# hongsukchoi/Pose2Mesh_RELEASE

Measured on NVIDIA H100. Metric: SMPL meshes/sec, higher is better.
Workload: dtype f32 (wgmma fp16x3 split, fp32 accumulate)

## Files before the change

### pose2mesh_release_b200/csrc/cheb_umma.cu

```cuda
#include <cuda.h>
#include <cuda_fp16.h>
#include <cuda_runtime.h>

#include <algorithm>
#include <cstdlib>
#include <cstring>
#include <vector>

#include "p2m_internal.h"

namespace p2m {

namespace {

constexpr int TILE_M = 128;
constexpr int FC = 32;
constexpr int A_BLOCK_BYTES = TILE_M * 128;
constexpr float W_SCALE = 64.f;
constexpr float W_INV_SCALE = 1.f / 64.f;

struct TileHeader {
  int n_rows;
  int h1;
  int nnz;
  int off_halo;
  int off_rp;
  int off_ent;
  int off_ord2;
  int bytes;
  int pad[8];
};
static_assert(sizeof(TileHeader) == 64, "header size");

inline int up16(int x) { return (x + 15) & ~15; }

constexpr int STG_ROW_BYTES = 544;

__device__ __forceinline__ uint32_t smem_u32(const void* p) { return (uint32_t)__cvta_generic_to_shared(p); }

__device__ __forceinline__ void mbar_init(uint32_t bar, uint32_t count) {
  asm volatile("mbarrier.init.shared::cta.b64 [%0], %1;" ::"r"(bar), "r"(count));
}
__device__ __forceinline__ void mbar_arrive(uint32_t bar) {
  asm volatile("mbarrier.arrive.shared::cta.b64 _, [%0];" ::"r"(bar) : "memory");
}
__device__ __forceinline__ void mbar_arrive_expect_tx(uint32_t bar, uint32_t bytes) {
  asm volatile("mbarrier.arrive.expect_tx.shared::cta.b64 _, [%0], %1;" ::"r"(bar), "r"(bytes) : "memory");
}
__device__ __forceinline__ bool mbar_try_wait(uint32_t bar, uint32_t parity) {
  uint32_t ok;
  asm volatile(
      "{\n\t.reg .pred p;\n\t"
      "mbarrier.try_wait.parity.shared::cta.b64 p, [%1], %2, %3;\n\t"
      "selp.u32 %0, 1, 0, p;\n\t}"
      : "=r"(ok)
      : "r"(bar), "r"(parity), "r"(20000u)
      : "memory");
  return ok != 0;
}
__device__ __forceinline__ unsigned long long global_ns() {
  unsigned long long t;
  asm volatile("mov.u64 %0, %globaltimer;" : "=l"(t));
  return t;
}
constexpr unsigned long long MBAR_TIMEOUT_NS = 2000000000ull;
__device__ __noinline__ void mbar_timeout(volatile int* abort_flag, int* status, int code) {
  *abort_flag = 1;
  *reinterpret_cast<volatile int*>(status) = code;
  __threadfence_system();
}
__device__ __forceinline__ void mbar_wait(uint32_t bar, uint32_t parity, volatile int* abort_flag, int* status,
                                          int code) {
  if (mbar_try_wait(bar, parity)) return;
  unsigned long long t0 = 0;
  for (unsigned spin = 0;; ++spin) {
#pragma unroll 1
    for (int it = 0; it < 64; ++it) {
      if (mbar_try_wait(bar, parity)) return;
    }
    if (*abort_flag) return;
    if ((spin & 63u) == 63u) {
      const unsigned long long t = global_ns();
      if (t0 == 0) t0 = t;
      else if (t - t0 > MBAR_TIMEOUT_NS) break;
    }
  }
  mbar_timeout(abort_flag, status, code);
}
template <unsigned SLEEP_NS = 200>
__device__ __forceinline__ void mbar_wait_relaxed(uint32_t bar, uint32_t parity, volatile int* abort_flag, int* status,
                                                  int code) {
  if (mbar_try_wait(bar, parity)) return;
  unsigned long long t0 = 0;
  for (unsigned spin = 0;; ++spin) {
#pragma unroll 1
    for (int it = 0; it < 16; ++it) {
      if (mbar_try_wait(bar, parity)) return;
      __nanosleep(SLEEP_NS);
    }
    if (*abort_flag) return;
    if ((spin & 255u) == 255u) {
      const unsigned long long t = global_ns();
      if (t0 == 0) t0 = t;
      else if (t - t0 > MBAR_TIMEOUT_NS) break;
    }
  }
  mbar_timeout(abort_flag, status, code);
}
__device__ __forceinline__ void fence_barrier_init() { asm volatile("fence.mbarrier_init.release.cluster;" ::: "memory"); }
// ... 141 lines not shown
__device__ __forceinline__ void split4(const float4& v, uint2& hi, uint2& lo) {
  __half2 h0 = __floats2half2_rn(v.x, v.y), h1 = __floats2half2_rn(v.z, v.w);
  float2 f0 = __half22float2(h0), f1 = __half22float2(h1);
  __half2 l0 = __floats2half2_rn(v.x - f0.x, v.y - f0.y), l1 = __floats2half2_rn(v.z - f1.x, v.w - f1.y);
  hi.x = *reinterpret_cast<uint32_t*>(&h0);
  hi.y = *reinterpret_cast<uint32_t*>(&h1);
  lo.x = *reinterpret_cast<uint32_t*>(&l0);
  lo.y = *reinterpret_cast<uint32_t*>(&l1);
}

struct KParams {
  const float* x;
  int in_unpool;
  int V, P, fin;
  int n_tiles;
  const unsigned char* meta;
  const int* meta_bytes;
  int meta_stride, max_h1;
  const unsigned char* wpack;
  const float* zero_row;
  EpiDev ep;
  int res_identity;
  const float* t1;
  const float* a_scale;
  long long ldy;
  int y_col0;
  float* y;
  int* status;
  long long* trace;
  int own_table;
  const float* head_wt;
  float* head_z;
  const unsigned char* apack;
  long long wslice_bytes;
  long long wblock_stride;
  int tma;
  CUtensorMap tm_x, tm_t1;
};

#ifdef P2M_UMMA_TRACE
__device__ __forceinline__ void trace_ev(const KParams& p, int role, int& n, int ev) {
  if (p.trace != nullptr && blockIdx.x == 0 && blockIdx.y == 0 && n < 512) {
    p.trace[role * 512 + n] = ((long long)ev << 48) | (clock64() & 0xFFFFFFFFFFFFll);
    ++n;
  }
}
#else
__device__ __forceinline__ void trace_ev(const KParams&, int, int&, int) {}
#endif

constexpr int W_PROD = 16;
constexpr int W_XLOAD = 16, N_XLOAD = 2, W_BLOAD = 18, W_EPI0 = 20;
constexpr int NUM_THREADS2 = 24 * 32;
constexpr int REGS_LAUNCH = 80, REGS_UTIL = 40, REGS_EPI = 120;
static_assert(128 * (REGS_EPI - REGS_LAUNCH) <= 128 * (REGS_LAUNCH - REGS_UTIL), "register pool balance");
static_assert(W_XLOAD % 4 == 0 && W_EPI0 % 4 == 0 && W_EPI0 - W_XLOAD == 4, "setmaxnreg works on aligned warpgroups");

template <int N>
__host__ __device__ constexpr int tile_rows() { return N == 128 ? 64 : TILE_M; }
template <int N, int NS, int XS, int MODE>
__global__ void __launch_bounds__(NUM_THREADS2, 1) k_cheb_conv_umma(const __grid_constant__ KParams p) {
  static_assert(N == 64 || N == 128, "one warpgroup holds the CTA's 128 x 64 or 64 x 128 accumulator in registers");
  constexpr int TM = tile_rows<N>();
  constexpr int RPT = TM / 64;
  constexpr int H = TM / 64;
  constexpr int ER = 16 * H;
  constexpr bool KT1 = (MODE == 1);
  constexpr bool plain = !KT1;
  constexpr bool XDIRECT = KT1 && NS >= 3;
  constexpr int A_BYTES = TM * 128;
  constexpr int B_BLOCK_BYTES = N * 128;
  constexpr int SLOT_BYTES = A_BYTES + B_BLOCK_BYTES;

  extern __shared__ __align__(1024) unsigned char smem_raw[];
  unsigned char* ring = smem_raw;
  float* Xs = reinterpret_cast<float*>(ring + NS * SLOT_BYTES);
  const size_t xs_stage_floats = (XDIRECT && TM == 64) ? 0 : (size_t)TM * FC;
  float* T1s = Xs + XS * xs_stage_floats;
  const size_t t1_stage_floats = (size_t)p.max_h1 * FC;
  unsigned char* meta_s =
      reinterpret_cast<unsigned char*>(T1s + (plain ? 0 : XS) * t1_stage_floats);
  uint64_t* bars = reinterpret_cast<uint64_t*>(meta_s + 2 * (size_t)p.meta_stride);
  uint64_t* b_ab_full = bars;
  uint64_t* b_ab_empty = b_ab_full + NS;
  uint64_t* b_x_full = b_ab_empty + NS;
  uint64_t* b_x_empty = b_x_full + XS;
  uint64_t* b_m_full = b_x_empty + XS;
  uint64_t* b_m_empty = b_m_full + 2;
  uint32_t* flags = reinterpret_cast<uint32_t*>(b_m_empty + 2);
  volatile int* abort_flag = reinterpret_cast<volatile int*>(flags + 1);
  float* ep_mul = reinterpret_cast<float*>(flags + 4);
  float* ep_add = ep_mul + N;
  constexpr int EC = 32;
  constexpr int STG_WARP_BYTES = N == 128 ? 16 * STG_ROW_BYTES : 32 * EC * 4;
  unsigned char* epi_stage =
      reinterpret_cast<unsigned char*>((reinterpret_cast<uintptr_t>(ep_add + N) + 127) & ~(uintptr_t)127);
  int* own_s = reinterpret_cast<int*>(epi_stage + 4 * STG_WARP_BYTES);
  float* head_w_s = reinterpret_cast<float*>(own_s + 4 * 32);
  uint64_t* b_res = reinterpret_cast<uint64_t*>(head_w_s);

  const int tid = threadIdx.x;
  const int warp = tid >> 5;
  const int lane = tid & 31;
  const int n_chunk = p.fin / FC;
  const int n_use = 3 * n_chunk;

  if (tid == 0) {
    for (int s = 0; s < NS; ++s) {
      mbar_init(smem_u32(b_ab_full + s), p.apack != nullptr ? 1 : W_PROD + 1);
      mbar_init(smem_u32(b_ab_empty + s), 4);
    }
    for (int s = 0; s < XS; ++s) {
      mbar_init(smem_u32(b_x_full + s), N_XLOAD * 32 + 1);
      mbar_init(smem_u32(b_x_empty + s), 1);
    }
    for (int s = 0; s < 2; ++s) {
      mbar_init(smem_u32(b_m_full + s), 1);
      mbar_init(smem_u32(b_m_empty + s), 1);
    }
    if (N == 128)
      for (int w = 0; w < 4; ++w) mbar_init(smem_u32(b_res + w), 1);
    *abort_flag = (smem_u32(ring) & 1023u) ? 1 : 0;
    if (*abort_flag) mbar_timeout(abort_flag, p.status, 100);
    fence_barrier_init();
  }
  const float a_scale = p.a_scale ? *p.a_scale : 1.f;
  const int ecol0 = (int)blockIdx.y * N;
  for (int n = threadIdx.x; n < N; n += NUM_THREADS2) {
    const float sc = (p.ep.scale ? p.ep.scale[ecol0 + n] : 1.f) / a_scale;
    const float sh = p.ep.scale ? p.ep.shift[ecol0 + n] : 0.f;
    const float bi = p.ep.bias ? p.ep.bias[ecol0 + n] : 0.f;
    ep_mul[n] = W_INV_SCALE * sc;
    ep_add[n] = fmaf(bi, p.ep.scale ? p.ep.scale[ecol0 + n] : 1.f, sh);
  }
  if (N == 64 && p.head_z != nullptr)
    for (int i = threadIdx.x; i < 64 * 12; i += NUM_THREADS2) head_w_s[i] = p.head_wt[i];
  __syncthreads();

  if (warp >= W_XLOAD && warp < W_EPI0) {
  asm volatile("setmaxnreg.dec.sync.aligned.u32 %0;" ::"n"(REGS_UTIL));
  if (warp >= W_XLOAD && warp < W_XLOAD + N_XLOAD) {
    if (p.apack == nullptr) {
      const int lt = tid - W_XLOAD * 32;
      const int lq = lt & 7, lrg = lt >> 3;
      const int my_tiles = (p.n_tiles - (int)blockIdx.x + (int)gridDim.x - 1) / (int)gridDim.x;
      if (lt == 32 && p.tma) {
        if (!XDIRECT) asm volatile("prefetch.tensormap [%0];" ::"l"(reinterpret_cast<uint64_t>(&p.tm_x)) : "memory");
        if (KT1) asm volatile("prefetch.tensormap [%0];" ::"l"(reinterpret_cast<uint64_t>(&p.tm_t1)) : "memory");
      }
      auto fetch_meta = [&](int itf) {
        const int pat = (blockIdx.x + itf * gridDim.x) % p.P;
        const int m = itf & 1;
        mbar_wait_relaxed(smem_u32(b_m_empty + m), ((itf >> 1) & 1) ^ 1, abort_flag, p.status, 1);
        const int mbytes = p.meta_bytes[pat];
        mbar_arrive_expect_tx(smem_u32(b_m_full + m), mbytes);
        bulk_g2s(smem_u32(meta_s + (size_t)m * p.meta_stride), p.meta + (size_t)pat * p.meta_stride, mbytes,
                 smem_u32(b_m_full + m));
      };
      if (lt == 0 && my_tiles > 0) fetch_meta(0);
      const uint32_t fin_bytes = (uint32_t)p.fin * 4u;
      const int sh = p.in_unpool ? 1 : 0;
      int g2 = 0;
      int ltn = 0;
      for (int it2 = 0; it2 < my_tiles; ++it2) {
        const int tile2 = blockIdx.x + it2 * gridDim.x;
        const long long mesh_row0 = (long long)(tile2 / p.P) * p.V;
        const int m2 = it2 & 1;
        mbar_wait_relaxed(smem_u32(b_m_full + m2), (it2 >> 1) & 1, abort_flag, p.status, 8);
        const unsigned char* mb2 = meta_s + (size_t)m2 * p.meta_stride;
        const TileHeader* hdr2 = reinterpret_cast<const TileHeader*>(mb2);
        const int* halo = reinterpret_cast<const int*>(mb2 + hdr2->off_halo);
        const int h1 = hdr2->h1;
        for (int c2 = 0; c2 < n_chunk; ++c2, ++g2) {
          const int xs2 = g2 % XS;
          mbar_wait_relaxed(smem_u32(b_x_empty + xs2), ((g2 / XS) & 1) ^ 1, abort_flag, p.status, 11);
          if (lt == 0) trace_ev(p, 4, ltn, 1);
          const uint32_t xbar = smem_u32(b_x_full + xs2);
          auto stage_rows = [&](uint32_t dbase, const char* sbase, int first, int n_rows, int shift) {
            for (int i0 = first + lrg; i0 < n_rows; i0 += 32) {
              int v[4];
#pragma unroll
              for (int u = 0; u < 4; ++u) v[u] = (i0 + 8 * u < n_rows) ? halo[i0 + 8 * u] : -2;
#pragma unroll
              for (int u = 0; u < 4; ++u) {
                if (v[u] != -2) {
                  const uint32_t srow = (uint32_t)max(v[u], 0) >> shift;
                  cp_async16_zfill(dbase + (i0 + 8 * u) * 128, sbase + (uint64_t)srow * (uint64_t)fin_bytes,
                                   v[u] >= 0 ? 16u : 0u);
                }
              }
            }
          };
          const char* t1_mesh =
              reinterpret_cast<const char*>(KT1 ? p.t1 + mesh_row0 * p.fin + c2 * FC + lq * 4 : nullptr);
          const char* x_mesh = reinterpret_cast<const char*>(p.x + (mesh_row0 >> sh) * p.fin + c2 * FC + lq * 4);
          const uint32_t t1_dst = smem_u32(T1s + xs2 * t1_stage_floats) + lq * 16;
          const uint32_t x_dst = smem_u32(Xs + xs2 * xs_stage_floats) + lq * 16;
          if (p.tma) {
            if (lt == 32) {
              const int own0 = tile2 * TM;
              mbar_arrive_expect_tx(xbar, (XDIRECT ? 0 : (p.in_unpool ? TM / 2 : TM) * 128) + (KT1 ? TM * 128 : 0));
              if (!XDIRECT)
                tma_load_2d(smem_u32(Xs + xs2 * xs_stage_floats), &p.tm_x, c2 * FC, p.in_unpool ? own0 >> 1 : own0, xbar);
              if (KT1) tma_load_2d(smem_u32(T1s + xs2 * t1_stage_floats), &p.tm_t1, c2 * FC, own0, xbar);
            }
            if (KT1) stage_rows(t1_dst, t1_mesh, TM, h1, 0);
          } else {
            if (KT1) stage_rows(t1_dst, t1_mesh, 0, h1, 0);
            if (!XDIRECT) stage_rows(x_dst, x_mesh, 0, TM, sh);
            if (lt == 32) mbar_arrive(xbar);
          }
          cp_async_arrive_noinc(xbar);
          if (lt == 0) trace_ev(p, 4, ltn, 2);
          if (lt == 0 && c2 == (n_chunk > 1 ? 1 : 0) && it2 + 1 < my_tiles) fetch_meta(it2 + 1);
        }
      }
    }
  } else if (warp == W_BLOAD) {
    if (lane == 0) {
      uint32_t ucnt = 0;
      int tn = 0;
      const int uses = plain ? n_chunk : n_use;
      for (int tile = blockIdx.x; tile < p.n_tiles; tile += gridDim.x) {
        for (int u = 0; u < uses; ++u, ++ucnt) {
          const int s = ucnt % NS;
          const uint32_t par = (ucnt / NS) & 1;
          mbar_wait_relaxed(smem_u32(b_ab_empty + s), par ^ 1, abort_flag, p.status, 4);
          trace_ev(p, 1, tn, 10 + u);
          const unsigned char* wsl = p.wpack + (size_t)blockIdx.y * (size_t)p.wslice_bytes;
          if (p.apack != nullptr) {
            mbar_arrive_expect_tx(smem_u32(b_ab_full + s), B_BLOCK_BYTES + A_BYTES);
            bulk_g2s(smem_u32(ring + s * SLOT_BYTES), p.apack + ((size_t)tile * uses + u) * A_BYTES, A_BYTES,
                     smem_u32(b_ab_full + s));
          } else {
            mbar_arrive_expect_tx(smem_u32(b_ab_full + s), B_BLOCK_BYTES);
          }
          bulk_g2s(smem_u32(ring + s * SLOT_BYTES + A_BYTES), wsl + (size_t)u * (size_t)p.wblock_stride, B_BLOCK_BYTES,
                   smem_u32(b_ab_full + s));
        }
      }
    }
  }
  } else if (warp >= W_EPI0) {
    asm volatile("setmaxnreg.inc.sync.aligned.u32 %0;" ::"n"(REGS_EPI));
    const int wq = warp - W_EPI0;
    constexpr int CPR = EC / 4;
    constexpr int RPI = 32 / CPR;
    const uint32_t stg = smem_u32(epi_stage) + (uint32_t)wq * STG_WARP_BYTES;
    const int prow = lane / CPR, pc = lane % CPR;
    constexpr int NP = ER / RPI;
    int colk[2];
#pragma unroll
    for (int k = 0; k < 2; ++k) colk[k] = (int)(((uint32_t)pc ^ (uint32_t)((k * RPI + prow) & 7)) << 2);
    const int trow = (lane >> 4) * 64 + wq * 16 + (lane & 15);
    const int uses = plain ? n_chunk : n_use;
    uint32_t ucnt = 0;
    int it = 0;
    int etn = 0;
    for (int tile = blockIdx.x; tile < p.n_tiles; tile += gridDim.x, ++it) {
      const int b = tile / p.P, pat = tile - b * p.P;
      const long long mesh0 = (long long)b * p.V;
      int* own_w = own_s + wq * 32;
      {
        int v;
        if (lane >= ER) {
          v = -1;
        } else if (p.own_table) {
          v = __ldg(reinterpret_cast<const int*>(p.meta + (size_t)pat * p.meta_stride + 64) + trow);
        } else {
          v = pat * TM + trow;
          if (v >= p.V) v = -1;
        }
        __syncwarp();
        own_w[lane] = v;
        __syncwarp();
      }
      int own_v[NP];
#pragma unroll
      for (int i = 0; i < NP; ++i) own_v[i] = own_w[i * RPI + prow];
      if (N == 128) {
        if (lane < ER) bulk_wait_read0();
        __syncwarp();
        if (p.ep.res != nullptr && p.res_identity) {
          const uint32_t rbar = smem_u32(b_res + wq);
          const int n_valid = __popc(__ballot_sync(0xFFFFFFFFu, lane < ER && own_w[lane] >= 0));
          if (lane == 0) mbar_arrive_expect_tx(rbar, (uint32_t)n_valid * (N * 4));
          __syncwarp();
          if (lane < ER && own_w[lane] >= 0) {
            const long long r = mesh0 + own_w[lane];
            bulk_g2s(stg + lane * STG_ROW_BYTES, p.ep.res + (p.ep.res_unpool ? (r >> 1) : r) * p.ep.res_F + ecol0, N * 4,
                     rbar);
          }
        }
      }
      if (p.ep.res != nullptr && (N == 64 || !p.res_identity)) {
        const int lpr = ((p.apack != nullptr ? N : p.ep.res_F) * 4 + 127) >> 7;
        for (int j = lane; j < ER * lpr; j += 32) {
          const int rr = j / lpr, ln = j - rr * lpr;
          const int vtx = own_w[rr];
          if (vtx >= 0) {
            const long long r = mesh0 + vtx;
            prefetch_l2(p.ep.res + (p.ep.res_unpool ? (r >> 1) : r) * p.ep.res_F + (p.apack != nullptr ? ecol0 : 0) + ln * 32);
          }
        }
      }
      float acc[2][32];
#pragma unroll
      for (int h = 0; h < 2; ++h)
#pragma unroll
        for (int j = 0; j < 32; ++j) acc[h][j] = 0.f;
      if (wq == 0 && lane == 0) trace_ev(p, 3, etn, 1);
      for (int u = 0; u < uses; ++u, ++ucnt) {
        const uint32_t s = ucnt % NS;
        if (wq == 0 && lane == 0) trace_ev(p, 3, etn, 4);
        mbar_wait(smem_u32(b_ab_full + s), (ucnt / NS) & 1, abort_flag, p.status, 6);
        if (wq == 0 && lane == 0) trace_ev(p, 3, etn, 5);
        const uint32_t a0 = smem_u32(ring + s * SLOT_BYTES);
        wg_fence();
#pragma unroll
        for (int h = 0; h < 2; ++h) {
          const uint64_t da = make_desc_sw128(a0 + (TM == 128 ? (uint32_t)h * (64 * 128) : 0u));
          const uint64_t db = make_desc_sw128(a0 + A_BYTES + (TM == 64 ? (uint32_t)h * (64 * 128) : 0u));
          wgmma_m64n64<0, 0>(acc[h], da + 0, db + 0);
          wgmma_m64n64<0, 0>(acc[h], da + 2, db + 2);
          wgmma_m64n64<0, 0>(acc[h], da + 4, db + 0);
          wgmma_m64n64<0, 0>(acc[h], da + 6, db + 2);
          wgmma_m64n64<0, 0>(acc[h], da + 0, db + 4);
          wgmma_m64n64<0, 0>(acc[h], da + 2, db + 6);
        }
        wg_commit();
        wg_wait0();
        __syncwarp();
        if (lane == 0) mbar_arrive(smem_u32(b_ab_empty + s));
      }
      if (wq == 0 && lane == 0) trace_ev(p, 3, etn, 2);
      auto stage_slab = [&](int cb) {
#pragma unroll
        for (int h = 0; h < H; ++h)
#pragma unroll
          for (int jj = 0; jj < 4; ++jj)
#pragma unroll
            for (int r = 0; r < 2; ++r) {
              const int lr = 16 * h + (lane >> 2) + 8 * r;
              const int cc = 8 * jj + 2 * (lane & 3);
              const int j = 4 * (cb / 8 + jj) + 2 * r;
              sts_f2(stg + lr * (EC * 4) + ((((uint32_t)(cc >> 2)) ^ (uint32_t)(lr & 7)) << 4) + (cc & 3) * 4,
                     acc[h][j], acc[h][j + 1]);
            }
        __syncwarp();
      };
      if (N == 64 && p.head_z != nullptr) {
        float z[12];
#pragma unroll
        for (int j = 0; j < 12; ++j) z[j] = 0.f;
#pragma unroll
        for (int cb = 0; cb < N; cb += 32) {
          stage_slab(cb);
#pragma unroll
          for (int c = 0; c < 8; ++c) {
            const float4 a = lds_f4(stg + lane * (EC * 4) + (((uint32_t)c ^ (uint32_t)(lane & 7)) << 4));
            const float av[4] = {a.x, a.y, a.z, a.w};
#pragma unroll
            for (int e = 0; e < 4; ++e) {
              const int n = cb + 4 * c + e;
              float t = fmaf(av[e], ep_mul[n], ep_add[n]);
              if (p.ep.relu) t = fmaxf(t, 0.f);
              const float4 w0 = *reinterpret_cast<const float4*>(head_w_s + n * 12);
              const float4 w1 = *reinterpret_cast<const float4*>(head_w_s + n * 12 + 4);
              const float4 w2 = *reinterpret_cast<const float4*>(head_w_s + n * 12 + 8);
              z[0] = fmaf(t, w0.x, z[0]); z[1] = fmaf(t, w0.y, z[1]); z[2] = fmaf(t, w0.z, z[2]); z[3] = fmaf(t, w0.w, z[3]);
              z[4] = fmaf(t, w1.x, z[4]); z[5] = fmaf(t, w1.y, z[5]); z[6] = fmaf(t, w1.z, z[6]); z[7] = fmaf(t, w1.w, z[7]);
              z[8] = fmaf(t, w2.x, z[8]); z[9] = fmaf(t, w2.y, z[9]); z[10] = fmaf(t, w2.z, z[10]); z[11] = fmaf(t, w2.w, z[11]);
            }
          }
          __syncwarp();
        }
        if (own_w[lane] >= 0) {
          float4* zr = reinterpret_cast<float4*>(p.head_z + (mesh0 + own_w[lane]) * 12);
          zr[0] = make_float4(z[0], z[1], z[2], z[3]);
          zr[1] = make_float4(z[4], z[5], z[6], z[7]);
          zr[2] = make_float4(z[8], z[9], z[10], z[11]);
        }
      } else if (N == 128) {
        const bool res_id = p.ep.res != nullptr && p.res_identity;
        if (res_id) mbar_wait(smem_u32(b_res + wq), (uint32_t)it & 1u, abort_flag, p.status, 12);
        if (wq == 0 && lane == 0) trace_ev(p, 3, etn, 21);
#pragma unroll
        for (int h = 0; h < 2; ++h)
#pragma unroll
          for (int jg = 0; jg < 8; ++jg) {
            const int n = 64 * h + 8 * jg + 2 * (lane & 3);
            const float2 mu = *reinterpret_cast<const float2*>(ep_mul + n);
            const float2 ad = *reinterpret_cast<const float2*>(ep_add + n);
#pragma unroll
            for (int r = 0; r < 2; ++r) {
              const int j = 4 * jg + 2 * r;
              const uint32_t a = stg + ((lane >> 2) + 8 * r) * STG_ROW_BYTES + n * 4;
              float o0 = fmaf(acc[h][j], mu.x, ad.x), o1 = fmaf(acc[h][j + 1], mu.y, ad.y);
              if (p.ep.relu) {
                o0 = fmaxf(o0, 0.f);
                o1 = fmaxf(o1, 0.f);
              }
              if (res_id) {
                const float2 rv = lds_f2(a);
                o0 += rv.x;
                o1 += rv.y;
              }
              sts_f2(a, o0, o1);
            }
          }
        if (p.ep.res != nullptr && !p.res_identity) {
          __syncwarp();
          const int gn = ecol0 + 4 * lane;
          for (int rr = 0; rr < ER; ++rr) {
            const int vtx = own_w[rr];
            if (vtx >= 0) {
              const long long r = mesh0 + vtx;
              const float* res_row = p.ep.res + (p.ep.res_unpool ? (r >> 1) : r) * p.ep.res_F;
              const uint32_t a = stg + rr * STG_ROW_BYTES + lane * 16;
              const float4 v = lds_f4(a);
              float o[4] = {v.x, v.y, v.z, v.w};
#pragma unroll
              for (int e = 0; e < 4; ++e) {
                const float l = __ldg(p.ep.lam + gn + e);
                o[e] += (1.f - l) * __ldg(res_row + __ldg(p.ep.i0 + gn + e)) + l * __ldg(res_row + __ldg(p.ep.i1 + gn + e));
              }
              sts_f4(a, make_float4(o[0], o[1], o[2], o[3]));
            }
          }
        }
        if (wq == 0 && lane == 0) trace_ev(p, 3, etn, 22);
        fence_async_proxy();
        __syncwarp();
        if (lane < ER) {
          if (own_w[lane] >= 0)
            bulk_s2g(p.y + (mesh0 + own_w[lane]) * p.ldy + p.y_col0 + ecol0, stg + lane * STG_ROW_BYTES, N * 4);
          bulk_commit();
        }
        if (wq == 0 && lane == 0) trace_ev(p, 3, etn, 23);
      } else {
#pragma unroll
        for (int cb = 0; cb < N; cb += 32) {
          stage_slab(cb);
          float4 mu_k[2], ad_k[2];
#pragma unroll
          for (int k = 0; k < 2; ++k) {
            mu_k[k] = *reinterpret_cast<const float4*>(ep_mul + cb + colk[k]);
            ad_k[k] = *reinterpret_cast<const float4*>(ep_add + cb + colk[k]);
          }
#pragma unroll
          for (int i = 0; i < NP; ++i) {
            const int rr = i * RPI + prow;
            const int n = cb + colk[i & 1];
            const int gn = ecol0 + n;
            const float4 a = lds_f4(stg + rr * (EC * 4) + (pc << 4));
            const int vtx = own_v[i];
            if (vtx >= 0) {
              const float4 mu = mu_k[i & 1], ad = ad_k[i & 1];
              float o[4] = {fmaf(a.x, mu.x, ad.x), fmaf(a.y, mu.y, ad.y), fmaf(a.z, mu.z, ad.z), fmaf(a.w, mu.w, ad.w)};
              if (p.ep.relu) {
#pragma unroll
                for (int e = 0; e < 4; ++e) o[e] = fmaxf(o[e], 0.f);
              }
              const long long r = mesh0 + vtx;
              if (p.ep.res != nullptr) {
                const float* res_row = p.ep.res + (p.ep.res_unpool ? (r >> 1) : r) * p.ep.res_F;
                if (p.res_identity) {
                  const float4 rv = __ldg(reinterpret_cast<const float4*>(res_row + gn));
                  o[0] += rv.x; o[1] += rv.y; o[2] += rv.z; o[3] += rv.w;
                } else {
#pragma unroll
                  for (int e = 0; e < 4; ++e) {
                    const float l = __ldg(p.ep.lam + gn + e);
                    o[e] += (1.f - l) * __ldg(res_row + __ldg(p.ep.i0 + gn + e)) + l * __ldg(res_row + __ldg(p.ep.i1 + gn + e));
                  }
                }
              }
              *reinterpret_cast<float4*>(p.y + r * p.ldy + p.y_col0 + gn) = make_float4(o[0], o[1], o[2], o[3]);
            }
          }
          __syncwarp();
        }
      }
    }
    if (N == 128 && lane < ER) bulk_wait0();
  } else {
    if (p.apack == nullptr) {
    const int q = tid & 7;
    const int rg = tid >> 3;
    const uint32_t t1s_a = smem_u32(T1s);
    const uint32_t ring_a = smem_u32(ring);
    const int my_tiles = (p.n_tiles - (int)blockIdx.x + (int)gridDim.x - 1) / (int)gridDim.x;
    const int n_stage = my_tiles * n_chunk;

    uint32_t row[RPT], re[RPT], ent_a = 0;
    int ptn = 0;
    uint32_t slot = 0, spar = 0;
    uint32_t so_f[RPT], so_s[RPT];
#pragma unroll
    for (int ps = 0; ps < RPT; ++ps) row[ps] = re[ps] = so_f[ps] = so_s[ps] = 0;
    const bool odd = (rg & 1) != 0;
    auto next_slot = [&]() {
      if (++slot == (uint32_t)NS) {
        slot = 0;
        spar ^= 1u;
      }
    };

    const int xsh = (p.tma && p.in_unpool) ? 1 : 0;
    const float* xp[RPT];
#pragma unroll
    for (int ps = 0; ps < RPT; ++ps) xp[ps] = nullptr;
    int it = 0, c = -1;
    for (int g = 0; g < n_stage; ++g) {
      if (++c == n_chunk) {
        c = 0;
        ++it;
      }
      const int m = it & 1;
      const int xs = g % XS;
      float4 xd[RPT];
#pragma unroll
      for (int ps = 0; ps < RPT; ++ps) {
        xd[ps] = make_float4(0.f, 0.f, 0.f, 0.f);
        if (XDIRECT && c != 0 && xp[ps]) xd[ps] = __ldg(reinterpret_cast<const float4*>(xp[ps] + c * FC));
      }
      if (tid == 0) trace_ev(p, 0, ptn, 1);
      mbar_wait(smem_u32(b_x_full + xs), (g / XS) & 1, abort_flag, p.status, 9);
      if (tid == 0) trace_ev(p, 0, ptn, 2);

      if (c == 0) {
        mbar_wait(smem_u32(b_m_full + m), (it >> 1) & 1, abort_flag, p.status, 8);
        const unsigned char* mb = meta_s + (size_t)m * p.meta_stride;
        const TileHeader* hdr = reinterpret_cast<const TileHeader*>(mb);
        const uint32_t mb_a = smem_u32(mb);
        const uint32_t rp_a = mb_a + hdr->off_rp, ord2_a = mb_a + hdr->off_ord2;
        ent_a = mb_a + hdr->off_ent;
#pragma unroll
        for (int ps = 0; ps < RPT; ++ps) {
// ... 67 lines not shown
      };
      float4 x[RPT], t1v[RPT], t2[RPT];
      if (NS < 3) {
#pragma unroll
        for (int ps = 0; ps < RPT; ++ps) x[ps] = lds_f4(xs_q + (row[ps] >> xsh) * 128);
        emit(x);
#pragma unroll
        for (int ps = 0; ps < RPT; ++ps) t1v[ps] = lds_f4(t1s_q + row[ps] * 128);
        emit(t1v);
#pragma unroll
        for (int ps = 0; ps < RPT; ++ps) t2[ps] = gather_row4(ent_a, re[ps] & 0xFFFFu, re[ps] >> 16, t1s_q);
        if (tid == 0) trace_ev(p, 0, ptn, 6);
#pragma unroll
        for (int ps = 0; ps < RPT; ++ps) t2[ps] = cheb_t2(t2[ps], x[ps]);
        emit(t2);
      } else {
#pragma unroll
        for (int ps = 0; ps < RPT; ++ps) t2[ps] = gather_row4(ent_a, re[ps] & 0xFFFFu, re[ps] >> 16, t1s_q);
#pragma unroll
        for (int ps = 0; ps < RPT; ++ps) x[ps] = XDIRECT ? xd[ps] : lds_f4(xs_q + (row[ps] >> xsh) * 128);
#pragma unroll
        for (int ps = 0; ps < RPT; ++ps) t1v[ps] = lds_f4(t1s_q + row[ps] * 128);
        if (tid == 0) trace_ev(p, 0, ptn, 6);
        {
          uint32_t s2 = slot + 2, p2 = spar;
          if (s2 >= (uint32_t)NS) {
            s2 -= (uint32_t)NS;
            p2 ^= 1u;
          }
          mbar_wait(smem_u32(b_ab_empty + s2), p2 ^ 1u, abort_flag, p.status, 10);
        }
        emit(x);
        emit(t1v);
#pragma unroll
        for (int ps = 0; ps < RPT; ++ps) t2[ps] = cheb_t2(t2[ps], x[ps]);
        emit(t2);
      }
      if (NS >= 3) {
        fence_async_proxy();
        __syncwarp();
        if ((tid & 31) == 0) {
#pragma unroll
          for (int k = 0; k < 3; ++k) mbar_arrive(smem_u32(b_ab_full + (slot0 + k) % NS));
        }
      }
      if (tid == 0) trace_ev(p, 0, ptn, 7);
      producer_barrier();
      if (tid == 0) trace_ev(p, 0, ptn, 8);
      if (tid == 0) mbar_arrive(smem_u32(b_x_empty + xs));
      if (tid == 0 && c == n_chunk - 1) mbar_arrive(smem_u32(b_m_empty + m));
    }
    }
  }
}

struct DwParams {
  const float* x;
  int in_unpool;
  int V, P, fin;
  int n_tiles;
  const unsigned char* meta;
  const int* meta_bytes;
  int meta_stride, max_h1;
  const float* g;
  int fout_total, m_off, m_cols;
  int chunk0;
  const float* a_scale;
  float* dw;
  int* status;
  const float* t1;
  int g_unpool;
  int swap;
  int tma;
  CUtensorMap tm_x, tm_t1;
};

__device__ __forceinline__ uint64_t make_desc_sw128_mn(uint32_t saddr, uint32_t lbo_bytes) {
  uint64_t d = 0;
  d |= (uint64_t)((saddr & 0x3FFFF) >> 4);
  d |= (uint64_t)((lbo_bytes >> 4) & 0x3FFF) << 16;
  d |= (uint64_t)(1024 >> 4) << 32;
  d |= (uint64_t)1 << 62;
  return d;
}

constexpr int DW_NS = 3;
constexpr int DW_G_BYTES = 4 * A_BLOCK_BYTES;

template <int XS>
__global__ void __launch_bounds__(NUM_THREADS2, 1) k_cheb_dw_umma(const __grid_constant__ DwParams p) {
  extern __shared__ __align__(1024) unsigned char smem_raw[];
  unsigned char* ring = smem_raw;
  unsigned char* gblk = ring + DW_NS * A_BLOCK_BYTES;
  float* Xs = reinterpret_cast<float*>(gblk + DW_G_BYTES);
  constexpr size_t xs_stage_floats = (size_t)TILE_M * FC;
  float* T1s = Xs + XS * xs_stage_floats;
  const size_t t1_stage_floats = (size_t)p.max_h1 * FC;
  unsigned char* meta_s = reinterpret_cast<unsigned char*>(T1s + XS * t1_stage_floats);
  uint64_t* bars = reinterpret_cast<uint64_t*>(meta_s + 2 * (size_t)p.meta_stride);
  uint64_t* b_t_full = bars;
  uint64_t* b_t_empty = b_t_full + DW_NS;
  uint64_t* b_x_full = b_t_empty + DW_NS;
  uint64_t* b_x_empty = b_x_full + XS;
  uint64_t* b_m_full = b_x_empty + XS;
  uint64_t* b_m_empty = b_m_full + 2;
  uint64_t* b_g_full = b_m_empty + 2;
// ... 386 lines not shown
}
size_t smem_bytes_for(int N, int NS, int XS, const TileBlobs& t, bool t1_given) {
  return smem_bytes_dims(N, NS, XS, t.max_h1, t.stride, t1_given);
}
constexpr size_t SMEM_LIMIT = 227 * 1024;
constexpr int CONV_N = 64;
constexpr int WIDE_N = 128;
inline int conv_n(int fout) { return fout % WIDE_N == 0 ? WIDE_N : CONV_N; }
const TileBlobs& conv_tiles(int N, const DevLevel& g, const TileSet* tiles) {
  if (tiles != nullptr) return N == WIDE_N ? tiles->m64 : *tiles;
  return N == WIDE_N ? g.meta64 : g.meta128;
}
struct ConvCfg {
  int ns, xs;
};
ConvCfg conv_cfg(int N, const TileBlobs& t, bool t1_given) {
  for (int ns = N == WIDE_N ? 6 : 3; ns >= 3; ns -= 3)
    for (int xs = 2; xs >= 1; --xs)
      if (smem_bytes_for(N, ns, xs, t, t1_given) <= SMEM_LIMIT) return {ns, xs};
  return {0, 0};
}

typedef CUresult (*TmapEncodeFn)(CUtensorMap*, CUtensorMapDataType, cuuint32_t, void*, const cuuint64_t*, const cuuint64_t*,
                                 const cuuint32_t*, const cuuint32_t*, CUtensorMapInterleave, CUtensorMapSwizzle,
                                 CUtensorMapL2promotion, CUtensorMapFloatOOBfill);
TmapEncodeFn tmap_encoder() {
  static TmapEncodeFn fn = [] {
    void* f = nullptr;
    cudaDriverEntryPointQueryResult q;
    if (cudaGetDriverEntryPoint("cuTensorMapEncodeTiled", &f, cudaEnableDefault, &q) != cudaSuccess ||
        q != cudaDriverEntryPointSuccess)
      f = nullptr;
    return reinterpret_cast<TmapEncodeFn>(f);
  }();
  return fn;
}
bool make_row_tmap(CUtensorMap* tm, const float* base, long long rows, int fin, int box_rows) {
  TmapEncodeFn enc = tmap_encoder();
  if (enc == nullptr || (reinterpret_cast<uintptr_t>(base) & 15u) != 0) return false;
  const cuuint64_t dims[2] = {(cuuint64_t)fin, (cuuint64_t)rows};
  const cuuint64_t strides[1] = {(cuuint64_t)fin * 4};
  const cuuint32_t box[2] = {(cuuint32_t)FC, (cuuint32_t)box_rows};
  const cuuint32_t estr[2] = {1, 1};
  return enc(tm, CU_TENSOR_MAP_DATA_TYPE_FLOAT32, 2, const_cast<float*>(base), dims, strides, box, estr,
             CU_TENSOR_MAP_INTERLEAVE_NONE, CU_TENSOR_MAP_SWIZZLE_NONE, CU_TENSOR_MAP_L2_PROMOTION_L2_128B,
             CU_TENSOR_MAP_FLOAT_OOB_FILL_NONE) == CUDA_SUCCESS;
}

template <int N, int NS, int XS, int MODE>
int check_launch_regs() {
  static int state = 0;
  if (state == 0) {
    cudaFuncAttributes fa;
    P2M_CUDA_OK(cudaFuncGetAttributes(&fa, k_cheb_conv_umma<N, NS, XS, MODE>));
    state = (fa.numRegs == REGS_LAUNCH) ? 1 : -1;
  }
  if (state < 0) {
    set_error("k_cheb_conv_umma was compiled with a register count other than the one its setmaxnreg split assumes");
    return P2M_ERR_CUDA;
  }
  return P2M_OK;
}

template <int N, int NS, int XS>
int launch_cfg(const UmmaConvArgs& a, int* status, const float* zero_row, int sm_count, cudaStream_t s) {
  constexpr int TM = tile_rows<N>();
  const DevLevel& g = *a.g;
  const TileBlobs& t = conv_tiles(N, g, a.tiles);
  const size_t smem = smem_bytes_for(N, NS, XS, t, !a.plain);
  auto kern = a.plain ? k_cheb_conv_umma<N, NS, XS, 0> : k_cheb_conv_umma<N, NS, XS, 1>;
  P2M_CUDA_OK(cudaFuncSetAttribute(kern, cudaFuncAttributeMaxDynamicSharedMemorySize, (int)smem));
  P2M_TRY((a.plain ? check_launch_regs<N, NS, XS, 0>() : check_launch_regs<N, NS, XS, 1>()));
  KParams p;
  p.x = a.x;
  p.in_unpool = a.in_unpool;
  p.V = g.V;
  p.P = t.n_pattern;
  p.fin = a.fin;
  p.meta = t.meta;
  p.meta_bytes = t.bytes;
  p.meta_stride = t.stride;
  p.max_h1 = t.max_h1;
  p.own_table = a.tiles != nullptr ? 1 : 0;
  p.n_tiles = a.batch * p.P;
  p.wpack = static_cast<const unsigned char*>(a.wpack);
  p.apack = nullptr;
  p.wslice_bytes = (long long)N * 128;
  p.wblock_stride = (long long)a.fout * 128;
  p.zero_row = zero_row;
  p.ep = to_dev(a.ep);
  p.res_identity = (a.ep.res != nullptr && a.ep.res_F == a.fout) ? 1 : 0;
  p.y = a.y;
  p.t1 = a.t1;
  p.a_scale = a.a_scale;
  p.ldy = a.ldy > 0 ? a.ldy : a.fout;
  p.y_col0 = a.y_col0;
  p.status = status;
  p.trace = a.trace;
  p.head_wt = a.fout == 64 ? a.head_wt : nullptr;
  p.head_z = a.fout == 64 ? a.head_z : nullptr;
  if (N == WIDE_N) {
    const bool y_ok = (reinterpret_cast<uintptr_t>(p.y) & 15u) == 0 && (p.ldy * 4) % 16 == 0 && (p.y_col0 * 4) % 16 == 0;
    const bool res_ok = !p.res_identity || ((reinterpret_cast<uintptr_t>(p.ep.res) & 15u) == 0 && (p.ep.res_F * 4) % 16 == 0);
    if (!y_ok || !res_ok) {
      set_error("umma_conv: the 128-column epilogue needs 16-byte aligned output and identity-residual rows");
      return P2M_ERR_INVALID;
    }
  }
  p.tma = 0;
  std::memset(&p.tm_x, 0, sizeof(p.tm_x));
  std::memset(&p.tm_t1, 0, sizeof(p.tm_t1));
  if (a.tiles == nullptr && g.V % TILE_M == 0 && g_umma_tma) {
    const long long rows = (long long)a.batch * g.V;
    bool ok = make_row_tmap(&p.tm_x, a.x, a.in_unpool ? rows / 2 : rows, a.fin, a.in_unpool ? TM / 2 : TM);
    if (ok && a.t1 != nullptr) ok = make_row_tmap(&p.tm_t1, a.t1, rows, a.fin, TM);
    p.tma = ok ? 1 : 0;
  }
  const int n_slices = a.fout / N;
  const dim3 grid(std::min(p.n_tiles, std::max(1, sm_count / n_slices)), n_slices);
  kern<<<grid, NUM_THREADS2, smem, s>>>(p);
  P2M_LAUNCH_OK();
  return P2M_OK;
}

int launch_n(const UmmaConvArgs& a, int* status, const float* zero_row, int sm_count, cudaStream_t s) {
  const int N = conv_n(a.fout);
  const ConvCfg c = conv_cfg(N, conv_tiles(N, *a.g, a.tiles), !a.plain);
  if (c.ns == 0) {
    set_error("umma_conv: tile family does not fit shared memory");
    return P2M_ERR_INVALID;
  }
  if (N == CONV_N)
    return c.xs == 2 ? launch_cfg<CONV_N, 3, 2>(a, status, zero_row, sm_count, s)
                     : launch_cfg<CONV_N, 3, 1>(a, status, zero_row, sm_count, s);
  if (c.ns == 6)
    return c.xs == 2 ? launch_cfg<WIDE_N, 6, 2>(a, status, zero_row, sm_count, s)
                     : launch_cfg<WIDE_N, 6, 1>(a, status, zero_row, sm_count, s);
  return c.xs == 2 ? launch_cfg<WIDE_N, 3, 2>(a, status, zero_row, sm_count, s)
                   : launch_cfg<WIDE_N, 3, 1>(a, status, zero_row, sm_count, s);
}

}

namespace {
void balance_store_halves(std::vector<unsigned short>* ord) {
  std::vector<unsigned short> q0, q1;
  for (unsigned short r : *ord) ((r & 4) ? q1 : q0).push_back(r);
  if (q0.size() != q1.size() || (q0.size() & 1)) return;
  size_t o = 0;
  for (size_t g = 0; g + 1 < q0.size(); g += 2) {
    (*ord)[o++] = q0[g];
    (*ord)[o++] = q0[g + 1];
    (*ord)[o++] = q1[g];
    (*ord)[o++] = q1[g + 1];
  }
}

bool make_indexed_blob(const std::vector<int>& own, int tm, const int* rowptr, const int* colidx, const float* val,
                       std::vector<int>* slot_of, std::vector<unsigned char>* blob, int* h1_out) {
  std::vector<int> halo(own);
  int n_rows = 0;
  for (int i = 0; i < tm; ++i)
    if (own[i] >= 0) {
      (*slot_of)[own[i]] = i;
      ++n_rows;
    }
  for (int i = 0; i < tm; ++i) {
    if (own[i] < 0) continue;
    for (int e = rowptr[own[i]]; e < rowptr[own[i] + 1]; ++e) {
      const int v = colidx[e];
      if ((*slot_of)[v] < 0) {
        (*slot_of)[v] = (int)halo.size();
        halo.push_back(v);
// ... 343 lines not shown
  return P2M_OK;
}

size_t umma_plain_pack_bytes(int N, int K) { return (size_t)(K / FC) * N * 128; }

__global__ void __launch_bounds__(256) k_pack_rows(const float* __restrict__ X, int M, int K, unsigned char* __restrict__ out) {
  const long long idx = (long long)blockIdx.x * blockDim.x + threadIdx.x;
  const int n_chunk = K / FC;
  const long long total = (long long)((M + TILE_M - 1) / TILE_M) * n_chunk * TILE_M * 8;
  if (idx >= total) return;
  const int j = (int)(idx & 7);
  const int row = (int)((idx >> 3) % TILE_M);
  const long long blk = (idx >> 3) / TILE_M;
  const int c = (int)(blk % n_chunk);
  const long long r = (blk / n_chunk) * TILE_M + row;
  __align__(16) __half h[8];
#pragma unroll
  for (int e = 0; e < 8; ++e) {
    const float v = (r < M) ? X[r * K + c * FC + (j & 3) * 8 + e] : 0.f;
    const __half hi = __float2half_rn(v);
    h[e] = (j < 4) ? hi : __float2half_rn(v - __half2float(hi));
  }
  *reinterpret_cast<uint4*>(out + (size_t)blk * A_BLOCK_BYTES + sw128_off(row, j)) = *reinterpret_cast<const uint4*>(h);
}
__global__ void __launch_bounds__(256) k_pack_w_sliced(const float* __restrict__ W, int n_real, int N, int K, int ns,
                                                       unsigned char* __restrict__ out) {
  const long long idx = (long long)blockIdx.x * blockDim.x + threadIdx.x;
  const int n_chunk = K / FC;
  const long long total = (long long)N * n_chunk * 8;
  if (idx >= total) return;
  const int j = (int)(idx & 7);
  const int nl = (int)((idx >> 3) % ns);
  const long long blk = (idx >> 3) / ns;
  const int c = (int)(blk % n_chunk);
  const int n = (int)(blk / n_chunk) * ns + nl;
  __align__(16) __half h[8];
#pragma unroll
  for (int e = 0; e < 8; ++e) {
    const float w = (n < n_real) ? W[(size_t)n * K + c * FC + (j & 3) * 8 + e] * W_SCALE : 0.f;
    const __half hi = __float2half_rn(w);
    h[e] = (j < 4) ? hi : __float2half_rn(w - __half2float(hi));
  }
  *reinterpret_cast<uint4*>(out + (size_t)blk * ns * 128 + sw128_off(nl, j)) = *reinterpret_cast<const uint4*>(h);
}
size_t umma_gemm_apack_bytes(int M, int K) { return (size_t)((M + TILE_M - 1) / TILE_M) * (K / FC) * A_BLOCK_BYTES; }
size_t umma_gemm_wpack_bytes(int N, int K) { return (size_t)(K / FC) * N * 128; }
bool umma_gemm_supported(int M, int N, int K) { return M > 0 && K >= FC && K % FC == 0 && N >= 64 && N % 64 == 0; }

namespace {
template <int N>
int launch_gemm_cfg(KParams p, int n_slices, int sm_count, cudaStream_t s) {
  constexpr int NS = 3;
  const size_t smem = smem_bytes_dims(N, NS, 1, 0, 0, false);
  auto kern = k_cheb_conv_umma<N, NS, 1, 0>;
  P2M_TRY((check_launch_regs<N, NS, 1, 0>()));
  P2M_CUDA_OK(cudaFuncSetAttribute(kern, cudaFuncAttributeMaxDynamicSharedMemorySize, (int)smem));
  p.wslice_bytes = (long long)umma_gemm_wpack_bytes(N, p.fin);
  p.wblock_stride = (long long)N * 128;
  const dim3 grid(std::min(p.n_tiles, sm_count), n_slices);
  kern<<<grid, NUM_THREADS2, smem, s>>>(p);
  P2M_LAUNCH_OK();
  return P2M_OK;
}
}

int launch_umma_gemm(const float* X, const float* W, int M, int N, int K, const Epilogue& ep, float* Y, void* apack,
                     void* wpack, int* status, int sm_count, cudaStream_t s, int n_real) {
  if (n_real <= 0 || n_real > N) n_real = N;
  if (!umma_gemm_supported(M, N, K) || (ep.res != nullptr && ep.res_F != N)) {
    set_error("umma_gemm: unsupported shape");
    return P2M_ERR_INVALID;
  }
  {
    const long long total = (long long)((M + TILE_M - 1) / TILE_M) * (K / FC) * TILE_M * 8;
    k_pack_rows<<<(unsigned)((total + 255) / 256), 256, 0, s>>>(X, M, K, static_cast<unsigned char*>(apack));
    P2M_LAUNCH_OK();
  }
  const int tiles = (M + TILE_M - 1) / TILE_M;
  const int ns = CONV_N;
  {
    const long long total = (long long)N * (K / FC) * 8;
    k_pack_w_sliced<<<(unsigned)((total + 255) / 256), 256, 0, s>>>(W, n_real, N, K, ns, static_cast<unsigned char*>(wpack));
    P2M_LAUNCH_OK();
  }
  KParams p;
  std::memset(&p, 0, sizeof(p));
  p.V = M;
  p.P = tiles;
  p.fin = K;
  p.n_tiles = tiles;
  p.wpack = static_cast<const unsigned char*>(wpack);
  p.apack = static_cast<const unsigned char*>(apack);
  p.ep = to_dev(ep);
  p.res_identity = (ep.res != nullptr) ? 1 : 0;
  p.ldy = N;
  p.y = Y;
  p.status = status;
  return launch_gemm_cfg<CONV_N>(p, N / ns, sm_count, s);
}

int launch_umma_pack_plain(const float* Bmat, long long ld_n, long long ld_k, int N, int K, void* wpack, cudaStream_t s) {
  const int total = (K / FC) * N * 8;
  k_pack_plain<<<(total + 255) / 256, 256, 0, s>>>(Bmat, ld_n, ld_k, N, K, static_cast<unsigned char*>(wpack));
  P2M_LAUNCH_OK();
  return P2M_OK;
}

size_t umma_wpack_bytes(int fin, int fout) { return (size_t)(fin / FC) * 3 * fout * 128; }

int launch_umma_pack_weights(const float* W, int fin, int fout, void* wpack, cudaStream_t s) {
  const int total = (fin / FC) * 3 * fout * 8;
  k_pack_weights<<<(total + 255) / 256, 256, 0, s>>>(W, fin, fout, static_cast<unsigned char*>(wpack));
  P2M_LAUNCH_OK();
// ... 26 lines not shown
```

Baseline: 11600.

## Ping-pong two MMA warpgroups for the 128-column conv kernel

For the N = 128 configuration the kernel gets a second consumer warpgroup, and the two groups take alternate tiles. A turn barrier orders their use of the smem ring, so one group's epilogue can overlap the other's wgmma mainloop. The residual prefetch into the staging buffer now waits on a new stage-free barrier and is started opportunistically during the mainloop. Register splits are retuned for the extra warpgroup, with producers lowered to 56, at the cost of tighter register budgets and more synchronisation complexity.

Result: faster. 11770 (median of 6 runs) (+1.4%).

```diff
diff --git a/pose2mesh_release_b200/csrc/cheb_umma.cu b/pose2mesh_release_b200/csrc/cheb_umma.cu
--- a/pose2mesh_release_b200/csrc/cheb_umma.cu
+++ b/pose2mesh_release_b200/csrc/cheb_umma.cu
@@ -55,6 +55,17 @@
       "selp.u32 %0, 1, 0, p;\n\t}"
       : "=r"(ok)
       : "r"(bar), "r"(parity), "r"(20000u)
+      : "memory");
+  return ok != 0;
+}
+__device__ __forceinline__ bool mbar_test_wait(uint32_t bar, uint32_t parity) {
+  uint32_t ok;
+  asm volatile(
+      "{\n\t.reg .pred p;\n\t"
+      "mbarrier.test_wait.parity.shared::cta.b64 p, [%1], %2;\n\t"
+      "selp.u32 %0, 1, 0, p;\n\t}"
+      : "=r"(ok)
+      : "r"(bar), "r"(parity)
       : "memory");
   return ok != 0;
 }
@@ -302,15 +313,29 @@
 constexpr int W_PROD = 16;
 constexpr int W_XLOAD = 16, N_XLOAD = 2, W_BLOAD = 18, W_EPI0 = 20;
 constexpr int NUM_THREADS2 = 24 * 32;
+template <int N>
+__host__ __device__ constexpr int conv_mma_groups() { return N == 128 ? 2 : 1; }
+template <int N>
+__host__ __device__ constexpr int conv_threads() { return (W_EPI0 + 4 * conv_mma_groups<N>()) * 32; }
 constexpr int REGS_LAUNCH = 80, REGS_UTIL = 40, REGS_EPI = 120;
+constexpr int REGS_LAUNCH_PP = 72, REGS_UTIL_PP = 40, REGS_EPI_PP = 120, REGS_PROD_PP = 56;
+template <int N>
+constexpr int conv_launch_regs() { return N == 128 ? REGS_LAUNCH_PP : REGS_LAUNCH; }
 static_assert(128 * (REGS_EPI - REGS_LAUNCH) <= 128 * (REGS_LAUNCH - REGS_UTIL), "register pool balance");
+static_assert(2 * 128 * (REGS_EPI_PP - REGS_LAUNCH_PP) <=
+                  128 * (REGS_LAUNCH_PP - REGS_UTIL_PP) + 4 * 128 * (REGS_LAUNCH_PP - REGS_PROD_PP),
+              "register pool balance (N = 128)");
+static_assert(conv_threads<128>() * REGS_LAUNCH_PP <= 65536 && conv_threads<128>() * (REGS_LAUNCH_PP + 8) > 65536,
+              "N = 128 launch register count");
 static_assert(W_XLOAD % 4 == 0 && W_EPI0 % 4 == 0 && W_EPI0 - W_XLOAD == 4, "setmaxnreg works on aligned warpgroups");
 
 template <int N>
 __host__ __device__ constexpr int tile_rows() { return N == 128 ? 64 : TILE_M; }
 template <int N, int NS, int XS, int MODE>
-__global__ void __launch_bounds__(NUM_THREADS2, 1) k_cheb_conv_umma(const __grid_constant__ KParams p) {
-  static_assert(N == 64 || N == 128, "one warpgroup holds the CTA's 128 x 64 or 64 x 128 accumulator in registers");
+__device__ __forceinline__ void cheb_conv_body(const KParams& p) {
+  static_assert(N == 64 || N == 128, "one warpgroup holds a tile's 128 x 64 or 64 x 128 accumulator in registers");
+  constexpr int NT = conv_threads<N>();
+  constexpr int NG = conv_mma_groups<N>();
   constexpr int TM = tile_rows<N>();
   constexpr int RPT = TM / 64;
   constexpr int H = TM / 64;
@@ -337,7 +362,9 @@
   uint64_t* b_x_empty = b_x_full + XS;
   uint64_t* b_m_full = b_x_empty + XS;
   uint64_t* b_m_empty = b_m_full + 2;
-  uint32_t* flags = reinterpret_cast<uint32_t*>(b_m_empty + 2);
+  uint64_t* b_stg_free = b_m_empty + 2;
+  uint64_t* b_turn = b_stg_free + 1;
+  uint32_t* flags = reinterpret_cast<uint32_t*>(b_turn + 1);
   volatile int* abort_flag = reinterpret_cast<volatile int*>(flags + 1);
   float* ep_mul = reinterpret_cast<float*>(flags + 4);
   float* ep_add = ep_mul + N;
@@ -368,15 +395,18 @@
       mbar_init(smem_u32(b_m_full + s), 1);
       mbar_init(smem_u32(b_m_empty + s), 1);
     }
-    if (N == 128)
+    if (N == 128) {
       for (int w = 0; w < 4; ++w) mbar_init(smem_u32(b_res + w), 1);
+      mbar_init(smem_u32(b_stg_free), 4);
+      mbar_init(smem_u32(b_turn), 1);
+    }
     *abort_flag = (smem_u32(ring) & 1023u) ? 1 : 0;
     if (*abort_flag) mbar_timeout(abort_flag, p.status, 100);
     fence_barrier_init();
   }
   const float a_scale = p.a_scale ? *p.a_scale : 1.f;
   const int ecol0 = (int)blockIdx.y * N;
-  for (int n = threadIdx.x; n < N; n += NUM_THREADS2) {
+  for (int n = threadIdx.x; n < N; n += NT) {
     const float sc = (p.ep.scale ? p.ep.scale[ecol0 + n] : 1.f) / a_scale;
     const float sh = p.ep.scale ? p.ep.shift[ecol0 + n] : 0.f;
     const float bi = p.ep.bias ? p.ep.bias[ecol0 + n] : 0.f;
@@ -384,11 +414,11 @@
     ep_add[n] = fmaf(bi, p.ep.scale ? p.ep.scale[ecol0 + n] : 1.f, sh);
   }
   if (N == 64 && p.head_z != nullptr)
-    for (int i = threadIdx.x; i < 64 * 12; i += NUM_THREADS2) head_w_s[i] = p.head_wt[i];
+    for (int i = threadIdx.x; i < 64 * 12; i += NT) head_w_s[i] = p.head_wt[i];
   __syncthreads();
 
   if (warp >= W_XLOAD && warp < W_EPI0) {
-  asm volatile("setmaxnreg.dec.sync.aligned.u32 %0;" ::"n"(REGS_UTIL));
+  asm volatile("setmaxnreg.dec.sync.aligned.u32 %0;" ::"n"(N == 128 ? REGS_UTIL_PP : REGS_UTIL));
   if (warp >= W_XLOAD && warp < W_XLOAD + N_XLOAD) {
     if (p.apack == nullptr) {
       const int lt = tid - W_XLOAD * 32;
@@ -492,8 +522,10 @@
     }
   }
   } else if (warp >= W_EPI0) {
-    asm volatile("setmaxnreg.inc.sync.aligned.u32 %0;" ::"n"(REGS_EPI));
-    const int wq = warp - W_EPI0;
+    asm volatile("setmaxnreg.inc.sync.aligned.u32 %0;" ::"n"(N == 128 ? REGS_EPI_PP : REGS_EPI));
+    const int wq = NG == 2 ? (warp - W_EPI0) & 3 : warp - W_EPI0;
+    const int grp = NG == 2 ? (warp - W_EPI0) >> 2 : 0;
+    const int trole = grp == 0 ? 3 : 5;
     constexpr int CPR = EC / 4;
     constexpr int RPI = 32 / CPR;
     const uint32_t stg = smem_u32(epi_stage) + (uint32_t)wq * STG_WARP_BYTES;
@@ -508,9 +540,13 @@
     int it = 0;
     int etn = 0;
     for (int tile = blockIdx.x; tile < p.n_tiles; tile += gridDim.x, ++it) {
+      if (NG == 2 && (it & 1) != grp) {
+        ucnt += uses;
+        continue;
+      }
       const int b = tile / p.P, pat = tile - b * p.P;
       const long long mesh0 = (long long)b * p.V;
-      int* own_w = own_s + wq * 32;
+      int* own_w = own_s + wq * 32 + grp * 16;
       {
         int v;
         if (lane >= ER) {
@@ -522,27 +558,26 @@
           if (v >= p.V) v = -1;
         }
         __syncwarp();
-        own_w[lane] = v;
+        if (lane < ER) own_w[lane] = v;
         __syncwarp();
       }
       int own_v[NP];
 #pragma unroll
       for (int i = 0; i < NP; ++i) own_v[i] = own_w[i * RPI + prow];
-      if (N == 128) {
-        if (lane < ER) bulk_wait_read0();
+      const bool res_id = N == 128 && p.ep.res != nullptr && p.res_identity;
+      bool stg_wait = N == 128 && it > 0;
+      auto fetch_residual = [&]() {
+        const uint32_t rbar = smem_u32(b_res + wq);
+        const int n_valid = __popc(__ballot_sync(0xFFFFFFFFu, lane < ER && own_w[lane] >= 0));
+        if (lane == 0) mbar_arrive_expect_tx(rbar, (uint32_t)n_valid * (N * 4));
         __syncwarp();
-        if (p.ep.res != nullptr && p.res_identity) {
-          const uint32_t rbar = smem_u32(b_res + wq);
-          const int n_valid = __popc(__ballot_sync(0xFFFFFFFFu, lane < ER && own_w[lane] >= 0));
-          if (lane == 0) mbar_arrive_expect_tx(rbar, (uint32_t)n_valid * (N * 4));
-          __syncwarp();
-          if (lane < ER && own_w[lane] >= 0) {
-            const long long r = mesh0 + own_w[lane];
-            bulk_g2s(stg + lane * STG_ROW_BYTES, p.ep.res + (p.ep.res_unpool ? (r >> 1) : r) * p.ep.res_F + ecol0, N * 4,
-                     rbar);
-          }
-        }
-      }
+        if (lane < ER && own_w[lane] >= 0) {
+          const long long r = mesh0 + own_w[lane];
+          bulk_g2s(stg + lane * STG_ROW_BYTES, p.ep.res + (p.ep.res_unpool ? (r >> 1) : r) * p.ep.res_F + ecol0, N * 4,
+                   rbar);
+        }
+      };
+      if (res_id && !stg_wait) fetch_residual();
       if (p.ep.res != nullptr && (N == 64 || !p.res_identity)) {
         const int lpr = ((p.apack != nullptr ? N : p.ep.res_F) * 4 + 127) >> 7;
         for (int j = lane; j < ER * lpr; j += 32) {
@@ -559,12 +594,14 @@
       for (int h = 0; h < 2; ++h)
 #pragma unroll
         for (int j = 0; j < 32; ++j) acc[h][j] = 0.f;
-      if (wq == 0 && lane == 0) trace_ev(p, 3, etn, 1);
+      if (wq == 0 && lane == 0) trace_ev(p, trole, etn, 1);
+      if (NG == 2 && it > 0) mbar_wait(smem_u32(b_turn), (uint32_t)(it - 1) & 1u, abort_flag, p.status, 14);
       for (int u = 0; u < uses; ++u, ++ucnt) {
         const uint32_t s = ucnt % NS;
-        if (wq == 0 && lane == 0) trace_ev(p, 3, etn, 4);
+        if (wq == 0 && lane == 0) trace_ev(p, trole, etn, 4);
         mbar_wait(smem_u32(b_ab_full + s), (ucnt / NS) & 1, abort_flag, p.status, 6);
-        if (wq == 0 && lane == 0) trace_ev(p, 3, etn, 5);
+        if (wq == 0 && lane == 0) trace_ev(p, trole, etn, 5);
+        if (NG == 2 && u == uses - 1 && wq == 0 && lane == 0) mbar_arrive(smem_u32(b_turn));
         const uint32_t a0 = smem_u32(ring + s * SLOT_BYTES);
         wg_fence();
 #pragma unroll
@@ -582,8 +619,17 @@
         wg_wait0();
         __syncwarp();
         if (lane == 0) mbar_arrive(smem_u32(b_ab_empty + s));
-      }
-      if (wq == 0 && lane == 0) trace_ev(p, 3, etn, 2);
+        if (res_id && stg_wait) {
+          const uint32_t par = (uint32_t)(it - 1) & 1u;
+          if (u == uses - 1) mbar_wait(smem_u32(b_stg_free), par, abort_flag, p.status, 13);
+          if (u == uses - 1 || __any_sync(0xFFFFFFFFu, mbar_test_wait(smem_u32(b_stg_free), par))) {
+            stg_wait = false;
+            if (wq == 0 && lane == 0) trace_ev(p, trole, etn, 3);
+            fetch_residual();
+          }
+        }
+      }
+      if (wq == 0 && lane == 0) trace_ev(p, trole, etn, 2);
       auto stage_slab = [&](int cb) {
 #pragma unroll
         for (int h = 0; h < H; ++h)
@@ -632,9 +678,9 @@
           zr[2] = make_float4(z[8], z[9], z[10], z[11]);
         }
       } else if (N == 128) {
-        const bool res_id = p.ep.res != nullptr && p.res_identity;
+        if (stg_wait) mbar_wait(smem_u32(b_stg_free), (uint32_t)(it - 1) & 1u, abort_flag, p.status, 13);
         if (res_id) mbar_wait(smem_u32(b_res + wq), (uint32_t)it & 1u, abort_flag, p.status, 12);
-        if (wq == 0 && lane == 0) trace_ev(p, 3, etn, 21);
+        if (wq == 0 && lane == 0) trace_ev(p, trole, etn, 21);
 #pragma unroll
         for (int h = 0; h < 2; ++h)
 #pragma unroll
@@ -679,7 +725,7 @@
             }
           }
         }
-        if (wq == 0 && lane == 0) trace_ev(p, 3, etn, 22);
+        if (wq == 0 && lane == 0) trace_ev(p, trole, etn, 22);
         fence_async_proxy();
         __syncwarp();
         if (lane < ER) {
@@ -687,7 +733,11 @@
             bulk_s2g(p.y + (mesh0 + own_w[lane]) * p.ldy + p.y_col0 + ecol0, stg + lane * STG_ROW_BYTES, N * 4);
           bulk_commit();
         }
-        if (wq == 0 && lane == 0) trace_ev(p, 3, etn, 23);
+        if (wq == 0 && lane == 0) trace_ev(p, trole, etn, 23);
+        if (lane < ER) bulk_wait_read0();
+        __syncwarp();
+        if (lane == 0) mbar_arrive(smem_u32(b_stg_free));
+        if (wq == 0 && lane == 0) trace_ev(p, trole, etn, 24);
       } else {
 #pragma unroll
         for (int cb = 0; cb < N; cb += 32) {
@@ -735,6 +785,7 @@
     }
     if (N == 128 && lane < ER) bulk_wait0();
   } else {
+    if (N == 128) asm volatile("setmaxnreg.dec.sync.aligned.u32 %0;" ::"n"(REGS_PROD_PP));
     if (p.apack == nullptr) {
     const int q = tid & 7;
     const int rg = tid >> 3;
@@ -908,6 +959,21 @@
     }
     }
   }
+}
+
+template <int N, int NS, int XS, int MODE>
+__global__ void __launch_bounds__(conv_threads<N>(), 1) k_cheb_conv_umma(const __grid_constant__ KParams p) {
+  static_assert(N == 64, "the N = 128 configuration is k_cheb_conv_pp");
+  cheb_conv_body<N, NS, XS, MODE>(p);
+}
+template <int NS, int XS, int MODE>
+__global__ void __launch_bounds__(conv_threads<128>(), 1) k_cheb_conv_pp(const __grid_constant__ KParams p) {
+  cheb_conv_body<128, NS, XS, MODE>(p);
+}
+template <int N, int NS, int XS, int MODE>
+constexpr auto conv_kernel() {
+  if constexpr (N == 128) return k_cheb_conv_pp<NS, XS, MODE>;
+  else return k_cheb_conv_umma<N, NS, XS, MODE>;
 }
 
 struct DwParams {
@@ -1400,11 +1466,11 @@
   static int state = 0;
   if (state == 0) {
     cudaFuncAttributes fa;
-    P2M_CUDA_OK(cudaFuncGetAttributes(&fa, k_cheb_conv_umma<N, NS, XS, MODE>));
-    state = (fa.numRegs == REGS_LAUNCH) ? 1 : -1;
+    P2M_CUDA_OK(cudaFuncGetAttributes(&fa, conv_kernel<N, NS, XS, MODE>()));
+    state = (fa.numRegs == conv_launch_regs<N>()) ? 1 : -1;
   }
   if (state < 0) {
-    set_error("k_cheb_conv_umma was compiled with a register count other than the one its setmaxnreg split assumes");
+    set_error("the conv kernel was compiled with a register count other than the one its setmaxnreg split assumes");
     return P2M_ERR_CUDA;
   }
   return P2M_OK;
@@ -1416,7 +1482,7 @@
   const DevLevel& g = *a.g;
   const TileBlobs& t = conv_tiles(N, g, a.tiles);
   const size_t smem = smem_bytes_for(N, NS, XS, t, !a.plain);
-  auto kern = a.plain ? k_cheb_conv_umma<N, NS, XS, 0> : k_cheb_conv_umma<N, NS, XS, 1>;
+  auto kern = a.plain ? conv_kernel<N, NS, XS, 0>() : conv_kernel<N, NS, XS, 1>();
   P2M_CUDA_OK(cudaFuncSetAttribute(kern, cudaFuncAttributeMaxDynamicSharedMemorySize, (int)smem));
   P2M_TRY((a.plain ? check_launch_regs<N, NS, XS, 0>() : check_launch_regs<N, NS, XS, 1>()));
   KParams p;
@@ -1466,7 +1532,7 @@
   }
   const int n_slices = a.fout / N;
   const dim3 grid(std::min(p.n_tiles, std::max(1, sm_count / n_slices)), n_slices);
-  kern<<<grid, NUM_THREADS2, smem, s>>>(p);
+  kern<<<grid, conv_threads<N>(), smem, s>>>(p);
   P2M_LAUNCH_OK();
   return P2M_OK;
 }
@@ -1916,13 +1982,13 @@
 int launch_gemm_cfg(KParams p, int n_slices, int sm_count, cudaStream_t s) {
   constexpr int NS = 3;
   const size_t smem = smem_bytes_dims(N, NS, 1, 0, 0, false);
-  auto kern = k_cheb_conv_umma<N, NS, 1, 0>;
+  auto kern = conv_kernel<N, NS, 1, 0>();
   P2M_TRY((check_launch_regs<N, NS, 1, 0>()));
   P2M_CUDA_OK(cudaFuncSetAttribute(kern, cudaFuncAttributeMaxDynamicSharedMemorySize, (int)smem));
   p.wslice_bytes = (long long)umma_gemm_wpack_bytes(N, p.fin);
   p.wblock_stride = (long long)N * 128;
   const dim3 grid(std::min(p.n_tiles, sm_count), n_slices);
-  kern<<<grid, NUM_THREADS2, smem, s>>>(p);
+  kern<<<grid, conv_threads<N>(), smem, s>>>(p);
   P2M_LAUNCH_OK();
   return P2M_OK;
 }
```
